# CarloLucibello/GraphNeuralNetworks.jl

Hardware: NVIDIA H100
Metric: edges/sec fwd+bwd GCNConv 128-dim on 100M-edge graph (higher is better)
Workload: dtype f32

## Files before the change

graphneuralnetworks.jl_b200/_lib.py:

```python
from __future__ import annotations

import ctypes as C
import os
import re

_HERE = os.path.dirname(os.path.abspath(__file__))
LIB_PATH = os.path.join(_HERE, "lib", "libgnnb200.so")
HEADER_PATH = os.path.join(os.path.dirname(_HERE), "include", "gnnb200.h")

OK, EINVAL, ESIZE, ECUDA, ENOMEM, EUNSUPPORTED, EINDEX = range(7)
COPY_XJ, W_MUL_XJ = 0, 1
SUM, MEAN, MAX, MIN = 0, 1, 2, 3
SRC, DST = 0, 1
DIR_OUT, DIR_IN, DIR_BOTH = 0, 1, 2
CODES_DIRECTED, CODES_DIRECTED_NOLOOP, CODES_UNDIRECTED, CODES_UNDIRECTED_NOLOOP, CODES_BIPARTITE = range(5)


class GNNBError(RuntimeError):

    def __init__(self, status: int, msg: str):
        super().__init__(f"libgnnb200 status {status}: {msg}")
        self.status = status


# ... 97 lines not shown
    "gnnb_edge_codes_sorted": (_int, [_int, _i64, _i64, _vp, _vp, _i64, _int, _vp, C.POINTER(_i64), _vp]),
    "gnnb_codes_member": (_int, [_vp, _i64, _vp, _i64, _vp, _vp]),
    "gnnb_sample_codes": (_int, [C.c_uint64, _vp, _i64, _i64, C.c_uint64, _vp, C.POINTER(_i64), _vp]),
    "gnnb_sample_positions_host": (_int, [_i32, _i64, _int, C.c_uint64, C.c_uint64, _vp, _i64, C.POINTER(_i64)]),
    "gnnb_propagate_host": (_int, [_vp, _int, _int, _int, _f32p, _f32p, _i64, _f32p]),
    "gnnb_gcn_propagate_host": (_int, [_vp, _int, _f32p, _f32p, _i64, _f32p]),
    "gnnb_linear2": (_int, [_f32p, _f32p, _f32p, _f32p, _int, _i64, _i64, _i64, _i64, _f32p, _vp]),
    "gnnb_linear2_bwd": (_int, [_f32p, _f32p, _f32p, _f32p, _f32p, _int, _i64, _i64, _i64, _i64, _f32p, _f32p, _f32p, _f32p, _f32p, _vp]),
    "gnnb_gat_logit_terms": (_int, [_f32p, _f32p, _i64, _i64, _i64, _f32p, _f32p, _vp]),
    "gnnb_gat_logit_terms_bwd": (_int, [_f32p, _f32p, _f32p, _f32p, _i64, _i64, _i64, _f32p, _f32p, _vp]),
    "gnnb_gcn_conv_step_host": (_int, [_vp, _vp, _vp, _vp, _int, _i64, _i64, _vp, _vp, _vp, _vp, _vp]),
    "gnnb_rmat_edges": (_int, [_i64, _i64, C.c_uint64, _vp, _vp, _vp]),
    "gnnb_rmat_edges_range": (_int, [_i64, _i64, _i64, C.c_uint64, _vp, _vp, _vp]),
    "gnnb_shard_builder_create": (_int, [C.POINTER(_vp), _i64, _int, _int, _int, C.POINTER(_i64), _vp]),
    "gnnb_shard_builder_add": (_int, [_vp, _vp, _vp, _i64, _int, _int, _vp]),
    "gnnb_shard_builder_finish": (_int, [_vp, _int, _int, C.POINTER(_vp), C.POINTER(_i64), C.POINTER(_i64), C.POINTER(_i64),
                                         C.POINTER(_i64), _vp]),
    "gnnb_degree_accumulate": (_int, [_vp, _vp, _i64, _int, _int, _i64, _vp, _vp]),
    "gnnb_balanced_relabel": (_int, [_vp, _i64, _int, _vp, _vp, _vp]),
    "gnnb_shard_builder_halo": (_int, [_vp, _int, _vp, _vp]),
    "gnnb_shard_builder_destroy": (_int, [_vp]),
    "gnnb_set_chunk_edges": (_int, [_int]),
    "gnnb_set_kernel_variant": (_int, [_int]),
}

for _name, (_res, _args) in _SIGS.items():
    _fn = getattr(lib, _name)
    _fn.restype = _res
    _fn.argtypes = _args


if os.environ.get("GNNB_KERNEL_VARIANT"):
    check(lib.gnnb_set_kernel_variant(int(os.environ["GNNB_KERNEL_VARIANT"])))


def device_count() -> int:
    return int(lib.gnnb_device_count())


def launch_count() -> int:
    return int(lib.gnnb_launch_count())


def version() -> str:
    return lib.gnnb_version().decode()
```

graphneuralnetworks.jl_b200/csrc/api.cu:

```cuda
#include "common.cuh"
#include <string.h>
#include <math_constants.h>

namespace gnnb {

static thread_local char t_err[512] = "";
std::atomic<int64_t> g_launches{0};

void set_error(const char* fmt, ...) {
    va_list ap;
    va_start(ap, fmt);
    vsnprintf(t_err, sizeof(t_err), fmt, ap);
    va_end(ap);
}

extern bool g_reference_kernels;
int edge_dot(gnnb_graph* g, const float* dout, const float* x, const float* cs, const float* ct, int64_t D,
             float* dw_coo, cudaStream_t st);
int maxmin_bwd(gnnb_graph* g, const float* w_plan_src, const float* x, const float* dout, const float* out_fwd,
               int64_t D, float* dx, cudaStream_t st);

__global__ void mul_vec_kernel(const float* __restrict__ a, const float* __restrict__ b, int64_t n, float* __restrict__ o) {
    int64_t i = (int64_t)blockIdx.x * blockDim.x + threadIdx.x;
    if (i < n) o[i] = a[i] * b[i];
}

__global__ void rmat_kernel(int64_t N, int64_t first, int64_t count, uint64_t seed, int scale, int64_t* __restrict__ src,
                            int64_t* __restrict__ dst) {
    const int64_t k = (int64_t)blockIdx.x * blockDim.x + threadIdx.x;
    if (k >= count) return;
    const int64_t id = first + k;
    const uint32_t TA = 9563013u, TB = 12750684u, TC = 15938355u;
    uint64_t s = 0, d = 0;
    for (uint64_t retry = 0;; ++retry) {
        uint64_t state = splitmix64(seed ^ splitmix64((uint64_t)id * 0x100000001B3ull + retry));
        s = 0; d = 0;
        for (int l = 0; l < scale; ++l) {
            state = splitmix64(state);
            const uint32_t u = (uint32_t)(state >> 40);
// ... 25 lines not shown

static int plan_weights(gnnb_graph* g, const Csr& c, int msg, const float* w, size_t ws2_off_floats, const float** out,
                        cudaStream_t st) {
    *out = nullptr;
    if (msg != GNNB_W_MUL_XJ || !w || g->E == 0) return GNNB_OK;
    GNNB_TRY(ensure_ws2(g, sizeof(float) * ((size_t)g->E + ws2_off_floats)));
    float* p = g->ws2 + ws2_off_floats;
    GNNB_TRY(permute_edge_values(c, g->E, w, 1, p, st));
    *out = p;
    return GNNB_OK;
}

extern "C" {

const char* gnnb_last_error(void) { return t_err; }
const char* gnnb_version(void) { return "gnnb200 0.1 sm_90a"; }
int gnnb_device_count(void) {
    int n = 0;
    if (cudaGetDeviceCount(&n) != cudaSuccess) { cudaGetLastError(); return 0; }
    return n;
}
int64_t gnnb_launch_count(void) { return g_launches.load(); }
int gnnb_set_kernel_variant(int v) {
    if (v != 0 && v != 12) GNNB_FAIL(GNNB_EINVAL, "kernel variant must be 0 (default) or 12 (reference kernels), got %d", v);
    gnnb::g_reference_kernels = v == 12;
    return GNNB_OK;
}

int gnnb_propagate(gnnb_graph_t g, int transposed, int msg, int aggr, const float* x, const float* w,
                   const float* cs, const float* ct, int64_t D, float* out, void* stream) {
    GNNB_TRY(check_common(g, msg, aggr, D, w));
    if (!x || !out) GNNB_FAIL(GNNB_EINVAL, "x/out is NULL");
    cudaStream_t st = (cudaStream_t)stream;
    GNNB_TRY(ensure_csr(g, transposed != 0, st));
    const Csr& c = transposed ? g->by_src : g->by_dst;
    SegArgs a;
    a.x = x; a.cs = cs; a.ct = ct; a.out = out; a.D = D; a.aggr = aggr;
    GNNB_TRY(plan_weights(g, c, msg, w, 0, &a.w, st));
    return seg_reduce(g, c, a, st);
}

int gnnb_propagate_bwd(gnnb_graph_t g, int msg, int aggr, const float* dout, const float* x, const float* w,
                       const float* cs, const float* ct, const float* out_fwd, int64_t D, float* dx, float* dw,
                       void* stream) {
    GNNB_TRY(check_common(g, msg, aggr, D, w));
    if (!dout) GNNB_FAIL(GNNB_EINVAL, "dout is NULL");
    cudaStream_t st = (cudaStream_t)stream;
    const bool ismax = aggr == GNNB_MAX || aggr == GNNB_MIN;
// ... 35 lines not shown
        if (!x) GNNB_FAIL(GNNB_EINVAL, "dw needs x");
        GNNB_TRY(edge_dot(g, dout, x, cs, gscale, D, dw, st));
    }
    return GNNB_OK;
}

int gnnb_gcn_propagate(gnnb_graph_t g, int transposed, const float* x, const float* w, const float* c,
                       int64_t D, float* out, void* stream) {
    if (!g) GNNB_FAIL(GNNB_EINVAL, "graph handle is NULL");
    if (g->n_src != g->n_dst) GNNB_FAIL(GNNB_ESIZE, "gcn_propagate needs num_src == num_dst");
    if (!c) {
        if (w) GNNB_FAIL(GNNB_EINVAL, "c is NULL: the plan-owned normalisation exists for unweighted graphs only");
        if (!x || !out) GNNB_FAIL(GNNB_EINVAL, "x/out is NULL");
        if (D <= 0) GNNB_FAIL(GNNB_ESIZE, "feature dimension must be positive (got %lld)", (long long)D);
        cudaStream_t st = (cudaStream_t)stream;
        GNNB_TRY(ensure_csr(g, transposed != 0, st));
        GNNB_TRY(ensure_gcn_scale(g, transposed != 0, st));
        const Csr& cc = transposed ? g->by_src : g->by_dst;
        SegArgs a;
        a.x = x; a.cs = g->gcn_c; a.es = cc.es; a.ct = g->gcn_c; a.out = out; a.D = D; a.aggr = GNNB_SUM;
        return seg_reduce(g, cc, a, st);
    }
    return gnnb_propagate(g, transposed, w ? GNNB_W_MUL_XJ : GNNB_COPY_XJ, GNNB_SUM, x, w, c, c, D, out, stream);
}

int gnnb_gcn_propagate_bipartite(gnnb_graph_t g, int transposed, const float* x, int64_t D, float* out, void* stream) {
    if (!g) GNNB_FAIL(GNNB_EINVAL, "graph handle is NULL");
    if (!x || !out) GNNB_FAIL(GNNB_EINVAL, "x/out is NULL");
    if (D <= 0) GNNB_FAIL(GNNB_ESIZE, "feature dimension must be positive (got %lld)", (long long)D);
    cudaStream_t st = (cudaStream_t)stream;
    GNNB_TRY(ensure_csr(g, transposed != 0, st));
    GNNB_TRY(ensure_bipartite_gcn_scale(g, transposed != 0, st));
    const Csr& cc = transposed ? g->by_src : g->by_dst;
    SegArgs a;
    a.x = x; a.out = out; a.D = D; a.aggr = GNNB_SUM;
    a.cs = transposed ? g->bip_c_dst : g->bip_c_src;
    a.es = transposed ? g->bip_es_src : g->bip_es_dst;
    a.ct = transposed ? g->bip_c_src : g->bip_c_dst;
    return seg_reduce(g, cc, a, st);
}

int gnnb_propagate_halo(gnnb_graph_t g, int msg, int aggr, const float* x_local, const float* x_halo,
                        int64_t n_local, const float* w, const float* cs, const float* ct, int64_t D, float* out,
                        void* stream) {
    GNNB_TRY(check_common(g, msg, aggr, D, w));
    if (!out) GNNB_FAIL(GNNB_EINVAL, "out is NULL");
// ... 165 lines not shown
```

graphneuralnetworks.jl_b200/csrc/common.cuh:

```cuda
#pragma once
#include <cuda_runtime.h>
#include <stdint.h>
#include <stdio.h>
#include <stdarg.h>
#include <atomic>
#include <mutex>
#include "../../include/gnnb200.h"

namespace gnnb {

void set_error(const char* fmt, ...);
extern std::atomic<int64_t> g_launches;

#define GNNB_CUDA(expr)                                                                   \
    do {                                                                                  \
        cudaError_t _e = (expr);                                                          \
        if (_e != cudaSuccess) {                                                          \
            ::gnnb::set_error("%s failed: %s (%s:%d)", #expr, cudaGetErrorString(_e),     \
                              __FILE__, __LINE__);                                        \
            return (_e == cudaErrorMemoryAllocation) ? GNNB_ENOMEM : GNNB_ECUDA;          \
        }                                                                                 \
    } while (0)

#define GNNB_TRY(expr)                 \
// ... 18 lines not shown

__host__ __device__ static inline uint64_t splitmix64(uint64_t x) {
    x += 0x9E3779B97F4A7C15ull;
    x = (x ^ (x >> 30)) * 0xBF58476D1CE4E5B9ull;
    x = (x ^ (x >> 27)) * 0x94D049BB133111EBull;
    return x ^ (x >> 31);
}

constexpr int kNumSMs = 132;

struct Csr {
    int32_t* rowptr = nullptr;
    int32_t* col = nullptr;
    int32_t* row = nullptr;
    int32_t* eid = nullptr;
    int32_t* long_rows = nullptr;
    int32_t n_long = 0;
    int32_t nrows = 0;
    float* invdeg = nullptr;
    int32_t* items = nullptr;
    int32_t n_items = 0;
    int32_t n_empty = -1;
    float* es = nullptr;
    bool built = false;
};

#ifdef __CUDACC__
__device__ __forceinline__ float fmax_nan(float a, float b) {
    float d;
    asm("max.NaN.f32 %0, %1, %2;" : "=f"(d) : "f"(a), "f"(b));
    return d;
}
__device__ __forceinline__ float softmax_shift(float Mn) { return Mn == -__int_as_float(0x7f800000) ? 0.f : Mn; }
#endif

}

struct gnnb_graph {
    int64_t E = 0;
    int32_t n_src = 0, n_dst = 0;
    int32_t chunk = 128;
    int device = 0;
    int32_t* coo_src = nullptr;
    int32_t* coo_dst = nullptr;
    gnnb::Csr by_dst;
    gnnb::Csr by_src;
    float* ws = nullptr;
    size_t ws_bytes = 0;
    float* ws2 = nullptr;
    size_t ws2_bytes = 0;
    float* gcn_c = nullptr;
    float* bip_c_src = nullptr;
    float* bip_c_dst = nullptr;
    float* bip_es_dst = nullptr;
    float* bip_es_src = nullptr;
    void* host_ws = nullptr;
    size_t host_ws_bytes = 0;
    std::mutex mu;
};

namespace gnnb {
int ensure_ws(gnnb_graph* g, size_t bytes);
int ensure_ws2(gnnb_graph* g, size_t bytes);
int ensure_csr(gnnb_graph* g, bool transposed, cudaStream_t st);
int ensure_invdeg(gnnb_graph* g, Csr& c, cudaStream_t st);
int ensure_items(gnnb_graph* g, const Csr& c, cudaStream_t st);
int ensure_gcn_scale(gnnb_graph* g, bool transposed, cudaStream_t st);
int ensure_bipartite_gcn_scale(gnnb_graph* g, bool transposed, cudaStream_t st);
int rsqrt_exact(float* d, int64_t n, cudaStream_t st);
int run_head_flags(const uint64_t* keys, int64_t E, int32_t* flags, cudaStream_t st);

struct SegArgs {
    const float* x = nullptr;
    const float* x2 = nullptr;
    int32_t split = 0;
    const float* w = nullptr;
    const float* cs = nullptr;
    const float* es = nullptr;
    const float* ct = nullptr;
    float* out = nullptr;
    int64_t D = 0;
    int aggr = GNNB_SUM;
};
int seg_reduce(gnnb_graph* g, const Csr& c, const SegArgs& a, cudaStream_t st);
int permute_edge_values(const Csr& c, int64_t E, const float* coo_vals, int64_t K, float* plan_vals,
                        cudaStream_t st);
int unpermute_edge_values(const Csr& c, int64_t E, const float* plan_vals, int64_t K,
                          float* coo_vals, cudaStream_t st);
}
```

graphneuralnetworks.jl_b200/csrc/plan.cu:

```cuda
#include "common.cuh"
#include <cub/cub.cuh>
#include <thrust/iterator/counting_iterator.h>
#include <thrust/iterator/transform_iterator.h>

namespace gnnb {

static int g_chunk_default = 128;

template <typename T>
__global__ void convert_index_kernel(const T* __restrict__ in, int64_t n, int64_t base, int64_t limit,
                                     int32_t* __restrict__ out, int* __restrict__ bad) {
    int64_t i = (int64_t)blockIdx.x * blockDim.x + threadIdx.x;
    if (i >= n) return;
    int64_t v = (int64_t)in[i] - base;
    if (v < 0 || v >= limit) {
        *bad = 1;
        v = 0;
    }
    out[i] = (int32_t)v;
}

__global__ void iota_kernel(int32_t* out, int64_t n, int32_t start) {
    int64_t i = (int64_t)blockIdx.x * blockDim.x + threadIdx.x;
    if (i < n) out[i] = start + (int32_t)i;
// ... 108 lines not shown
                                    const int32_t* __restrict__ eid, int64_t E, const int32_t* __restrict__ pos,
                                    const int32_t* __restrict__ newid, const int32_t* __restrict__ map,
                                    int32_t* __restrict__ nrow, int32_t* __restrict__ ncol,
                                    int32_t* __restrict__ neid) {
    int64_t k = (int64_t)blockIdx.x * blockDim.x + threadIdx.x;
    if (k >= E) return;
    const int32_t p = pos[k];
    if (pos[k + 1] == p) return;
    nrow[p] = map[row[k]];
    ncol[p] = map[col[k]];
    neid[p] = newid[eid[k]];
}

__global__ void bernoulli_keep_kernel(int64_t n, double p, uint64_t key, uint8_t* __restrict__ keep) {
    int64_t i = (int64_t)blockIdx.x * blockDim.x + threadIdx.x;
    if (i >= n) return;
    const double u = (double)(splitmix64(key + (uint64_t)i) >> 11) * 0x1.0p-53;
    keep[i] = (u < p) ? 0 : 1;
}

static void free_csr(Csr& c) {
    cudaFree(c.rowptr); cudaFree(c.col); cudaFree(c.row); cudaFree(c.eid);
    cudaFree(c.long_rows); cudaFree(c.invdeg); cudaFree(c.items); cudaFree(c.es);
    c = Csr();
}

static int alloc_csr(Csr& c, int64_t E, int32_t nrows, int32_t chunk) {
    c.nrows = nrows;
    GNNB_CUDA(cudaMalloc(&c.rowptr, sizeof(int32_t) * ((size_t)nrows + 1)));
    GNNB_CUDA(cudaMalloc(&c.col, sizeof(int32_t) * (size_t)(E > 0 ? E : 1)));
    GNNB_CUDA(cudaMalloc(&c.row, sizeof(int32_t) * (size_t)(E > 0 ? E : 1)));
    GNNB_CUDA(cudaMalloc(&c.eid, sizeof(int32_t) * (size_t)(E > 0 ? E : 1)));
    GNNB_CUDA(cudaMalloc(&c.long_rows, sizeof(int32_t) * (size_t)(E / chunk + 2)));
    return GNNB_OK;
}

static int find_long_rows(Csr& c, int32_t chunk, cudaStream_t st) {
    int32_t* d_count = nullptr;
    GNNB_CUDA(cudaMalloc(&d_count, sizeof(int32_t)));
    GNNB_CUDA(cudaMemsetAsync(d_count, 0, sizeof(int32_t), st));
    if (c.nrows > 0) {
        long_rows_kernel<<<(unsigned)ceil_div(c.nrows, 256), 256, 0, st>>>(c.rowptr, c.nrows, chunk,
                                                                           c.long_rows, d_count);
        GNNB_LAUNCHED();
    }
    GNNB_CUDA(cudaMemcpyAsync(&c.n_long, d_count, sizeof(int32_t), cudaMemcpyDeviceToHost, st));
// ... 376 lines not shown
```

graphneuralnetworks.jl_b200/csrc/seglean.cu:

```cuda
#include "common.cuh"
#include "segwalk.cuh"
#include <cub/cub.cuh>
#include <math_constants.h>

namespace gnnb {

struct LeanParams {
    const int4* __restrict__ items;
    const int32_t* __restrict__ col;
    const int32_t* __restrict__ row;
    const int32_t* __restrict__ rowptr;
    const float* __restrict__ es;
    const float* __restrict__ cs;
    const float* __restrict__ w;
    const float* __restrict__ ct;
    const float* __restrict__ x;
    const float* __restrict__ x2;
    float* __restrict__ out;
    float* __restrict__ ws;
    int32_t n_items;
    int32_t split;
    int32_t mean;
    float sign;
};

namespace {

__device__ __forceinline__ int chunk_items(const int32_t* __restrict__ rowptr, const int32_t* __restrict__ row, int64_t k,
                                           int C, int E, int nchunks, int4 out[3]) {
    const ChunkBounds b = chunk_bounds(rowptr, row, k, C, E, nchunks);
    if (b.e_begin >= b.e_end) return 0;
    int n = 0;
    int mb = b.e_begin, me = b.e_end;
    if (b.head_partial) {
        const int r0 = __ldg(row + b.e_begin);
        const int re0 = __ldg(rowptr + r0 + 1);
        const int hb = re0 < b.e_end ? re0 : b.e_end;
        out[n++] = make_int4(b.e_begin, hb, (int)(2 * k), 0);
        mb = hb;
    }
    int4 tail = make_int4(0, 0, -1, 0);
    if (mb < b.e_end && b.tail_partial) {
        const int r1 = __ldg(row + b.e_end - 1);
        const int rs1 = __ldg(rowptr + r1);
        const int tb = rs1 > mb ? rs1 : mb;
        me = tb;
// ... 33 lines not shown
    const int64_t r0 = ((int64_t)blockIdx.x * (blockDim.x >> 5) + (threadIdx.x >> 5)) * 32;
    const int64_t r = r0 + lane;
    const bool empty = r < nrows && __ldg(rowptr + r) == __ldg(rowptr + r + 1);
    unsigned m = __ballot_sync(0xffffffffu, empty);
    const float4 v4 = make_float4(v, v, v, v);
    while (m) {
        const int j = __ffs(m) - 1;
        m &= m - 1;
        float* base = out + (size_t)(r0 + j) * D;
        if ((D & 3) == 0 && (reinterpret_cast<uintptr_t>(base) & 15) == 0) {
            for (int64_t f = (int64_t)lane * 4; f < D; f += 128) *reinterpret_cast<float4*>(base + f) = v4;
        } else {
            for (int64_t f = lane; f < D; f += 32) base[f] = v;
        }
    }
}

__global__ void gather_scale_kernel(const int32_t* __restrict__ col, int64_t E, const float* __restrict__ c,
                                    float* __restrict__ es) {
    const int64_t e = (int64_t)blockIdx.x * blockDim.x + threadIdx.x;
    if (e < E) es[e] = __ldg(c + __ldg(col + e));
}

__device__ __forceinline__ float4 f4(float v) { return make_float4(v, v, v, v); }

constexpr int AG_SUM = 0, AG_MEAN = 1, AG_MAX = 2;

template <int SMODE, bool HAS_W, int AGG>
__device__ __forceinline__ float lcomb1(float acc, float v, float s1, float s2, float sign) {
    float m = v;
    if (SMODE != 0) m = __fmul_rn(m, s1);
    if (HAS_W) m = __fmul_rn(m, s2);
    if (AGG == AG_MAX) return fmax_nan(acc, __fmul_rn(m, sign));
    return __fadd_rn(acc, m);
}
template <int SMODE, bool HAS_W, int AGG>
__device__ __forceinline__ float4 lcomb(float4 a, float4 v, float s1, float s2, float sign) {
    return make_float4(lcomb1<SMODE, HAS_W, AGG>(a.x, v.x, s1, s2, sign), lcomb1<SMODE, HAS_W, AGG>(a.y, v.y, s1, s2, sign),
                       lcomb1<SMODE, HAS_W, AGG>(a.z, v.z, s1, s2, sign), lcomb1<SMODE, HAS_W, AGG>(a.w, v.w, s1, s2, sign));
}

template <int KV, int SMODE, bool HAS_W, int HALO, int AGG>
__global__ void __launch_bounds__(256, 4) seg_lean_kernel(const LeanParams p) {
    constexpr unsigned FULL = 0xffffffffu;
    constexpr int U = 8 / KV;
    constexpr int64_t STRIDE = (int64_t)KV * 128;
    const int lane = threadIdx.x & 31;
    const int item = blockIdx.x * 8 + (threadIdx.x >> 5);
    if (item >= p.n_items) return;
    const int4 it = __ldg(p.items + item);
    const int e_end = it.y;
    const bool partial = __any_sync(FULL, it.z >= 0);
    const float neutral = (AGG == AG_MAX) ? -CUDART_INF_F : 0.f;
    const float* const xl = p.x + lane * 4;
    const float* const x2l = HALO ? p.x2 + lane * 4 - (int64_t)p.split * STRIDE : nullptr;

    auto load_lane = [&](int e0, int& c, int& r, float& s1, float& s2, bool& last) {
        const int my = e0 + lane;
        c = 0; r = 0; s1 = 1.f; s2 = 1.f; last = false;
        if (my < e_end) {
            c = __ldg(p.col + my);
            r = __ldg(p.row + my);
            if (SMODE == 1) s1 = __ldg(p.es + my);
            if (HAS_W) s2 = __ldg(p.w + my);
            last = (my + 1 == e_end) || (__ldg(p.row + my + 1) != r);
            if (SMODE == 2) s1 = __ldg(p.cs + c);
        }
    };

    float4 acc[KV];
#pragma unroll
    for (int i = 0; i < KV; ++i) acc[i] = f4(neutral);

    int e = it.x;
    int c_n, r_n;
    float s1_n, s2_n;
    bool last_n;
    load_lane(e, c_n, r_n, s1_n, s2_n, last_n);
    bool more = true;
    while (more) {
        const int c_l = c_n, r_l = r_n;
        const float s1_l = s1_n, s2_l = s2_n;
        const unsigned vmask = __ballot_sync(FULL, e + lane < e_end);
        const unsigned bmask = partial ? 0u : __ballot_sync(FULL, last_n);
        float sc_l = 1.f, dg_l = 1.f;
        if (!partial && e + lane < e_end) {
            if (p.ct) sc_l = __ldg(p.ct + r_l);
            if (AGG == AG_MEAN) dg_l = (float)(__ldg(p.rowptr + r_l + 1) - __ldg(p.rowptr + r_l));
        }
        if (AGG == AG_MAX) sc_l *= p.sign;
        more = __any_sync(FULL, e + 32 < e_end);
        if (more) load_lane(e + 32, c_n, r_n, s1_n, s2_n, last_n);
#pragma unroll 1
        for (int j0 = 0; j0 < 32 && (vmask >> j0) != 0u; j0 += U) {
            float4 v[U][KV];
#pragma unroll
            for (int u = 0; u < U; ++u) {
                const int cj = __shfl_sync(FULL, c_l, j0 + u);
                const bool second = HALO != 0 && cj >= p.split;
                const float* xr = (second ? x2l : xl) + (int64_t)cj * STRIDE;
                if ((vmask >> (j0 + u)) & 1u) {
#pragma unroll
                    for (int i = 0; i < KV; ++i) v[u][i] = __ldg(reinterpret_cast<const float4*>(xr + i * 128));
                }
            }
#pragma unroll
            for (int u = 0; u < U; ++u) {
                const float s1 = (SMODE != 0) ? __shfl_sync(FULL, s1_l, j0 + u) : 1.f;
                const float s2 = HAS_W ? __shfl_sync(FULL, s2_l, j0 + u) : 1.f;
                if ((vmask >> (j0 + u)) & 1u) {
#pragma unroll
                    for (int i = 0; i < KV; ++i) acc[i] = lcomb<SMODE, HAS_W, AGG>(acc[i], v[u][i], s1, s2, p.sign);
                }
                if ((bmask >> (j0 + u)) & 1u) {
                    const int rj = __shfl_sync(FULL, r_l, j0 + u);
                    const float sc = __shfl_sync(FULL, sc_l, j0 + u);
                    float* o = p.out + (int64_t)rj * STRIDE + lane * 4;
                    if (AGG == AG_MEAN) {
                        const float dg = __shfl_sync(FULL, dg_l, j0 + u);
#pragma unroll
                        for (int i = 0; i < KV; ++i)
                            acc[i] = make_float4(__fdiv_rn(acc[i].x, dg), __fdiv_rn(acc[i].y, dg),
                                                 __fdiv_rn(acc[i].z, dg), __fdiv_rn(acc[i].w, dg));
                    }
#pragma unroll
                    for (int i = 0; i < KV; ++i) {
                        const float4 res = make_float4(acc[i].x * sc, acc[i].y * sc, acc[i].z * sc, acc[i].w * sc);
                        *reinterpret_cast<float4*>(o + i * 128) = res;
                        acc[i] = f4(neutral);
                    }
                }
            }
        }
        e += 32;
    }
    if (partial) {
        float* o = p.ws + (int64_t)it.z * STRIDE + lane * 4;
#pragma unroll
        for (int i = 0; i < KV; ++i) *reinterpret_cast<float4*>(o + i * 128) = acc[i];
    }
}

struct MaxBwdParams {
    const int4* __restrict__ items;
    const int32_t* __restrict__ col;
    const int32_t* __restrict__ row;
    const float* __restrict__ w;
    const float* __restrict__ x;
    const float* __restrict__ dout;
    const float* __restrict__ of;
    float* __restrict__ dx;
// ... 132 lines not shown
        LP(cub::DeviceScan::ExclusiveSum(nullptr, tmp_bytes, counts, offs, nchunks + 1, st));
        LP(cudaMalloc(&tmp, tmp_bytes ? tmp_bytes : 1));
        LP(cub::DeviceScan::ExclusiveSum(tmp, tmp_bytes, counts, offs, nchunks + 1, st));
        count_empty_rows_kernel<<<(unsigned)ceil_div((int64_t)c.nrows, 256), 256, 0, st>>>(c.rowptr, c.nrows, d_empty);
        int32_t n_items = 0, n_empty = 0;
        LP(cudaMemcpyAsync(&n_items, offs + nchunks, sizeof(int32_t), cudaMemcpyDeviceToHost, st));
        LP(cudaMemcpyAsync(&n_empty, d_empty, sizeof(int32_t), cudaMemcpyDeviceToHost, st));
        LP(cudaStreamSynchronize(st));
        LP(cudaMalloc(&items, sizeof(int4) * (size_t)(n_items > 0 ? n_items : 1)));
        item_emit_kernel<<<(unsigned)ceil_div(nchunks, 256), 256, 0, st>>>(c.rowptr, c.row, g->chunk, (int)g->E, nchunks, offs, items);
        LP(cudaGetLastError());
        LP(cudaStreamSynchronize(st));
        g_launches.fetch_add(4, std::memory_order_relaxed);
        mc.n_items = n_items;
        mc.n_empty = n_empty;
        mc.items = reinterpret_cast<int32_t*>(items);
        items = nullptr;
#undef LP
    } while (0);
    cudaFree(counts); cudaFree(offs); cudaFree(d_empty); cudaFree(tmp); cudaFree(items);
    return status;
}

int ensure_gcn_scale(gnnb_graph* g, bool transposed, cudaStream_t st) {
    Csr& c = transposed ? g->by_src : g->by_dst;
    if (g->gcn_c != nullptr && (c.es != nullptr || g->E == 0)) return GNNB_OK;
    if (g->gcn_c == nullptr) {
        float* buf = nullptr;
        GNNB_CUDA(cudaMalloc(&buf, sizeof(float) * (size_t)(g->n_dst > 0 ? g->n_dst : 1)));
        int rc = gnnb_gcn_norm(g, nullptr, buf, st);
        if (rc != GNNB_OK) { cudaFree(buf); return rc; }
        GNNB_CUDA(cudaStreamSynchronize(st));
        std::lock_guard<std::mutex> lock(g->mu);
        if (g->gcn_c == nullptr) g->gcn_c = buf; else cudaFree(buf);
    }
    if (c.es == nullptr && g->E > 0) {
        float* es = nullptr;
        GNNB_CUDA(cudaMalloc(&es, sizeof(float) * (size_t)g->E));
        gather_scale_kernel<<<(unsigned)ceil_div(g->E, 256), 256, 0, st>>>(c.col, g->E, g->gcn_c, es);
        GNNB_LAUNCHED();
        GNNB_CUDA(cudaStreamSynchronize(st));
        std::lock_guard<std::mutex> lock(g->mu);
        if (c.es == nullptr) c.es = es; else cudaFree(es);
    }
    return GNNB_OK;
}

int ensure_bipartite_gcn_scale(gnnb_graph* g, bool transposed, cudaStream_t st) {
    float*& es_slot = transposed ? g->bip_es_src : g->bip_es_dst;
    if (g->bip_c_src != nullptr && g->bip_c_dst != nullptr && (es_slot != nullptr || g->E == 0)) return GNNB_OK;
    GNNB_TRY(ensure_csr(g, true, st));
    if (g->bip_c_src == nullptr || g->bip_c_dst == nullptr) {
        float *cs = nullptr, *cd = nullptr;
        GNNB_CUDA(cudaMalloc(&cs, sizeof(float) * (size_t)(g->n_src > 0 ? g->n_src : 1)));
        GNNB_CUDA(cudaMalloc(&cd, sizeof(float) * (size_t)(g->n_dst > 0 ? g->n_dst : 1)));
        int rc = gnnb_degree(g, GNNB_DIR_OUT, nullptr, cs, st);
        if (rc == GNNB_OK) rc = gnnb_degree(g, GNNB_DIR_IN, nullptr, cd, st);
        if (rc == GNNB_OK) rc = rsqrt_exact(cs, g->n_src, st);
        if (rc == GNNB_OK) rc = rsqrt_exact(cd, g->n_dst, st);
        if (rc != GNNB_OK) { cudaFree(cs); cudaFree(cd); return rc; }
        GNNB_CUDA(cudaStreamSynchronize(st));
        std::lock_guard<std::mutex> lock(g->mu);
        if (g->bip_c_src == nullptr) { g->bip_c_src = cs; g->bip_c_dst = cd; } else { cudaFree(cs); cudaFree(cd); }
    }
    if (es_slot == nullptr && g->E > 0) {
        const Csr& c = transposed ? g->by_src : g->by_dst;
        float* es = nullptr;
// ... 11 lines not shown
    if (a.D != 128 && a.D != 256 && a.D != 512) return GNNB_EUNSUPPORTED;
    if ((reinterpret_cast<uintptr_t>(a.x) & 15) || (reinterpret_cast<uintptr_t>(a.x2) & 15) ||
        (reinterpret_cast<uintptr_t>(a.out) & 15))
        return GNNB_EUNSUPPORTED;
    const bool ismax = (a.aggr == GNNB_MAX || a.aggr == GNNB_MIN);
    const int agg = ismax ? AG_MAX : (a.aggr == GNNB_MEAN ? AG_MEAN : AG_SUM);
    const int smode = (a.cs == nullptr) ? 0 : (a.es != nullptr ? 1 : 2);
    const bool halo = a.x2 != nullptr;
    if (agg != AG_SUM && (smode != 0 || halo)) return GNNB_EUNSUPPORTED;
    GNNB_TRY(ensure_items(g, c, st));
    if (c.n_empty > 0) {
        const float v = a.aggr == GNNB_MAX ? -HUGE_VALF : (a.aggr == GNNB_MIN ? HUGE_VALF : 0.f);
        fill_empty_rows_warp_kernel<<<(unsigned)ceil_div((int64_t)c.nrows, 256), 256, 0, st>>>(c.rowptr, c.nrows, a.out, a.D, v);
        GNNB_LAUNCHED();
    }
    LeanParams p;
    p.items = reinterpret_cast<const int4*>(c.items);
    p.n_items = c.n_items;
    p.col = c.col; p.row = c.row; p.rowptr = c.rowptr;
    p.es = a.es; p.cs = a.cs; p.w = a.w; p.ct = a.ct;
    p.x = a.x; p.x2 = a.x2; p.split = a.split; p.out = a.out; p.ws = ws;
    p.mean = (a.aggr == GNNB_MEAN);
    p.sign = (a.aggr == GNNB_MIN) ? -1.f : 1.f;
    if (p.n_items == 0) return GNNB_OK;
    const int use_halo = halo ? 1 : 0;
    int rc;
    if (a.D == 128) rc = launch_lean1<1>(p, smode, a.w != nullptr, use_halo, agg, st);
    else if (a.D == 256) rc = launch_lean1<2>(p, smode, a.w != nullptr, use_halo, agg, st);
    else rc = launch_lean1<4>(p, smode, a.w != nullptr, use_halo, agg, st);
    return rc;
}

int seg_fixup_sum(const Csr& c, int64_t E, int chunk, int64_t D, float* ws, float* out, cudaStream_t st);
int maxmin_bwd_lean(gnnb_graph* g, const float* w_plan_src, const float* x, const float* dout, const float* out_fwd,
                    int64_t D, float* dx, cudaStream_t st) {
    if (D != 128 && D != 256 && D != 512) return GNNB_EUNSUPPORTED;
    if ((reinterpret_cast<uintptr_t>(x) & 15) || (reinterpret_cast<uintptr_t>(dout) & 15) ||
        (reinterpret_cast<uintptr_t>(out_fwd) & 15) || (reinterpret_cast<uintptr_t>(dx) & 15))
        return GNNB_EUNSUPPORTED;
    const Csr& c = g->by_src;
    if (g->E == 0) return GNNB_EUNSUPPORTED;
    GNNB_TRY(ensure_items(g, c, st));
    if (c.n_empty > 0) {
        fill_empty_rows_warp_kernel<<<(unsigned)ceil_div((int64_t)c.nrows, 256), 256, 0, st>>>(c.rowptr, c.nrows, dx, D, 0.f);
        GNNB_LAUNCHED();
    }
    MaxBwdParams p;
    p.items = reinterpret_cast<const int4*>(c.items);
    p.n_items = c.n_items;
    p.col = c.col; p.row = c.row; p.w = w_plan_src; p.x = x; p.dout = dout; p.of = out_fwd; p.dx = dx; p.ws = nullptr;
    if (c.n_long > 0) {
        GNNB_TRY(ensure_ws(g, (size_t)2 * ceil_div(g->E, g->chunk) * D * sizeof(float)));
// ... 16 lines not shown
```

include/gnnb200.h:

```cpp
#ifndef GNNB200_H
#define GNNB200_H

#include <stdint.h>

#ifdef __cplusplus
extern "C" {
#endif

typedef enum {
    GNNB_OK = 0,
    GNNB_EINVAL = 1,
    GNNB_ESIZE = 2,
    GNNB_ECUDA = 3,
    GNNB_ENOMEM = 4,
    GNNB_EUNSUPPORTED = 5,
    GNNB_EINDEX = 6
} gnnb_status;

typedef enum {
    GNNB_COPY_XJ = 0,
    GNNB_W_MUL_XJ = 1
} gnnb_msg;

typedef enum { GNNB_SUM = 0, GNNB_MEAN = 1, GNNB_MAX = 2, GNNB_MIN = 3 } gnnb_aggr;
// ... 30 lines not shown

int gnnb_degree(gnnb_graph_t g, int dir, const float* w, float* out, void* stream);

int gnnb_gather(gnnb_graph_t g, int which, const float* x, int64_t D, float* out, void* stream);

int gnnb_scatter(gnnb_graph_t g, int which, int aggr, const float* m, int64_t D, float* out,
                 void* stream);

int gnnb_propagate(gnnb_graph_t g, int transposed, int msg, int aggr, const float* x,
                   const float* w, const float* cs, const float* ct, int64_t D, float* out,
                   void* stream);

int gnnb_propagate_bwd(gnnb_graph_t g, int msg, int aggr, const float* dout, const float* x,
                       const float* w, const float* cs, const float* ct, const float* out_fwd,
                       int64_t D, float* dx, float* dw, void* stream);

int gnnb_softmax_edge_neighbors(gnnb_graph_t g, const float* e, int64_t K, float* out, void* stream);
int gnnb_softmax_edge_neighbors_bwd(gnnb_graph_t g, const float* alpha, const float* dalpha,
                                    int64_t K, float* de, void* stream);

int gnnb_gcn_norm(gnnb_graph_t g, const float* w, float* c_out, void* stream);
int gnnb_gcn_propagate(gnnb_graph_t g, int transposed, const float* x, const float* w,
                       const float* c, int64_t D, float* out, void* stream);
int gnnb_gcn_propagate_bipartite(gnnb_graph_t g, int transposed, const float* x, int64_t D, float* out, void* stream);

int gnnb_gat_aggregate(gnnb_graph_t g, const float* Wx, const float* el, const float* er,
                       int64_t C, int64_t H, float slope, float* out, float* alpha,
                       float* seg_max, float* seg_sum, void* stream);
int gnnb_gat_aggregate_bwd(gnnb_graph_t g, const float* Wx, const float* el, const float* er,
                           const float* seg_max, const float* seg_sum, const float* out_fwd,
                           const float* dout, int64_t C, int64_t H, float slope, float* dWx, float* del,
                           float* der, void* stream);

int gnnb_gat_logit_terms(const float* Wx, const float* a, int64_t N, int64_t C, int64_t H, float* el, float* er, void* stream);
int gnnb_gat_logit_terms_bwd(const float* Wx, const float* a, const float* del, const float* der, int64_t N, int64_t C,
                             int64_t H, float* dWx_accum, float* da, void* stream);

int gnnb_linear(const float* x, const float* W, const float* bias, int relu, int64_t N, int64_t Din,
                int64_t Dout, float* y, void* stream);
int gnnb_linear_bwd(const float* dy, const float* y, const float* x, const float* W, int relu, int64_t N,
                    int64_t Din, int64_t Dout, float* dpre_ws, float* dx, float* dW, float* db, void* stream);
int gnnb_linear_relu_mask(const float* x, const float* W, const float* bias, int64_t N, int64_t Din, int64_t Dout, float* y,
                          uint32_t* mask, void* stream);
int gnnb_linear_bwd_mask(const float* dy, const uint32_t* mask, const float* x, const float* W, int64_t N, int64_t Din,
                         int64_t Dout, float* dx, float* dW, float* db, void* stream);
int gnnb_linear2(const float* x1, const float* x2, const float* W, const float* bias, int relu, int64_t N, int64_t Din1,
// ... 133 lines not shown
```

Measured before the change: 2.096 billion.

## Pin high-degree source rows in L2 with cache-policy hints during GCN gather

During GCN scale setup, the code counts how often each source row is gathered, picks a threshold so the hottest rows fit in about half of L2, and marks those edges by setting the sign bit of the per-edge scale. In the 128-dim lean seg-reduce kernel, gathers of hot rows use an evict_last policy, cold rows use evict_first, and output stores use evict_first. A follow-up kernel resets the hot rows to evict_normal. The aim is to cut DRAM traffic from repeated gathers on power-law graphs, in exchange for a one-time count/sort/sync setup, an extra launch per propagate, and a sign-bit encoding trick on the edge scales.

```diff
diff --git a/graphneuralnetworks.jl_b200/_lib.py b/graphneuralnetworks.jl_b200/_lib.py
--- a/graphneuralnetworks.jl_b200/_lib.py
+++ b/graphneuralnetworks.jl_b200/_lib.py
@@ -143,6 +143,7 @@
     "gnnb_shard_builder_destroy": (_int, [_vp]),
     "gnnb_set_chunk_edges": (_int, [_int]),
     "gnnb_set_kernel_variant": (_int, [_int]),
+    "gnnb_gcn_hot_rows": (_int, [_vp, _int, _vp, _i64, C.POINTER(_i64), C.POINTER(C.c_int32), _vp]),
 }
 
 for _name, (_res, _args) in _SIGS.items():
diff --git a/graphneuralnetworks.jl_b200/csrc/api.cu b/graphneuralnetworks.jl_b200/csrc/api.cu
--- a/graphneuralnetworks.jl_b200/csrc/api.cu
+++ b/graphneuralnetworks.jl_b200/csrc/api.cu
@@ -15,6 +15,7 @@
 }
 
 extern bool g_reference_kernels;
+extern bool g_l2_policy_forced;
 int edge_dot(gnnb_graph* g, const float* dout, const float* x, const float* cs, const float* ct, int64_t D,
              float* dw_coo, cudaStream_t st);
 int maxmin_bwd(gnnb_graph* g, const float* w_plan_src, const float* x, const float* dout, const float* out_fwd,
@@ -86,8 +87,10 @@
 }
 int64_t gnnb_launch_count(void) { return g_launches.load(); }
 int gnnb_set_kernel_variant(int v) {
-    if (v != 0 && v != 12) GNNB_FAIL(GNNB_EINVAL, "kernel variant must be 0 (default) or 12 (reference kernels), got %d", v);
+    if (v != 0 && v != 12 && v != 14)
+        GNNB_FAIL(GNNB_EINVAL, "kernel variant must be 0 (default), 12 (reference kernels) or 14 (L2 policy at every size), got %d", v);
     gnnb::g_reference_kernels = v == 12;
+    gnnb::g_l2_policy_forced = v == 14;
     return GNNB_OK;
 }
 
@@ -169,6 +172,14 @@
         return seg_reduce(g, cc, a, st);
     }
     return gnnb_propagate(g, transposed, w ? GNNB_W_MUL_XJ : GNNB_COPY_XJ, GNNB_SUM, x, w, c, c, D, out, stream);
+}
+
+int gnnb_gcn_hot_rows(gnnb_graph_t g, int transposed, int32_t* rows_host, int64_t capacity, int64_t* num_rows,
+                      int32_t* threshold, void* stream) {
+    if (!g) GNNB_FAIL(GNNB_EINVAL, "graph handle is NULL");
+    if (g->n_src != g->n_dst) GNNB_FAIL(GNNB_ESIZE, "gcn_hot_rows needs num_src == num_dst");
+    if (capacity < 0) GNNB_FAIL(GNNB_ESIZE, "capacity must be >= 0");
+    return gcn_hot_rows(g, transposed != 0, rows_host, capacity, num_rows, threshold, (cudaStream_t)stream);
 }
 
 int gnnb_gcn_propagate_bipartite(gnnb_graph_t g, int transposed, const float* x, int64_t D, float* out, void* stream) {
diff --git a/graphneuralnetworks.jl_b200/csrc/common.cuh b/graphneuralnetworks.jl_b200/csrc/common.cuh
--- a/graphneuralnetworks.jl_b200/csrc/common.cuh
+++ b/graphneuralnetworks.jl_b200/csrc/common.cuh
@@ -64,6 +64,9 @@
     int32_t n_items = 0;
     int32_t n_empty = -1;
     float* es = nullptr;
+    int32_t hot_min = 0;
+    int32_t* hot_rows = nullptr;
+    int32_t n_hot = 0;
     bool built = false;
 };
 
@@ -108,6 +111,8 @@
 int ensure_invdeg(gnnb_graph* g, Csr& c, cudaStream_t st);
 int ensure_items(gnnb_graph* g, const Csr& c, cudaStream_t st);
 int ensure_gcn_scale(gnnb_graph* g, bool transposed, cudaStream_t st);
+int gcn_hot_rows(gnnb_graph* g, bool transposed, int32_t* rows_host, int64_t capacity, int64_t* num_rows,
+                 int32_t* threshold, cudaStream_t st);
 int ensure_bipartite_gcn_scale(gnnb_graph* g, bool transposed, cudaStream_t st);
 int rsqrt_exact(float* d, int64_t n, cudaStream_t st);
 int run_head_flags(const uint64_t* keys, int64_t E, int32_t* flags, cudaStream_t st);
diff --git a/graphneuralnetworks.jl_b200/csrc/plan.cu b/graphneuralnetworks.jl_b200/csrc/plan.cu
--- a/graphneuralnetworks.jl_b200/csrc/plan.cu
+++ b/graphneuralnetworks.jl_b200/csrc/plan.cu
@@ -154,6 +154,7 @@
 static void free_csr(Csr& c) {
     cudaFree(c.rowptr); cudaFree(c.col); cudaFree(c.row); cudaFree(c.eid);
     cudaFree(c.long_rows); cudaFree(c.invdeg); cudaFree(c.items); cudaFree(c.es);
+    cudaFree(c.hot_rows);
     c = Csr();
 }
 
diff --git a/graphneuralnetworks.jl_b200/csrc/seglean.cu b/graphneuralnetworks.jl_b200/csrc/seglean.cu
--- a/graphneuralnetworks.jl_b200/csrc/seglean.cu
+++ b/graphneuralnetworks.jl_b200/csrc/seglean.cu
@@ -22,6 +22,7 @@
     int32_t split;
     int32_t mean;
     float sign;
+    int32_t l2hint;
 };
 
 namespace {
@@ -101,9 +102,58 @@
     if (e < E) es[e] = __ldg(c + __ldg(col + e));
 }
 
+__global__ void count_gathers_kernel(const int32_t* __restrict__ col, int64_t E, int32_t* __restrict__ cnt) {
+    const int64_t e = (int64_t)blockIdx.x * blockDim.x + threadIdx.x;
+    if (e < E) atomicAdd(cnt + __ldg(col + e), 1);
+}
+__global__ void flag_hot_kernel(const int32_t* __restrict__ col, int64_t E, const int32_t* __restrict__ cnt, int32_t t,
+                                float* __restrict__ es) {
+    const int64_t e = (int64_t)blockIdx.x * blockDim.x + threadIdx.x;
+    if (e < E && __ldg(cnt + __ldg(col + e)) >= t) es[e] = __uint_as_float(__float_as_uint(es[e]) | 0x80000000u);
+}
+__global__ void list_hot_kernel(const int32_t* __restrict__ cnt, int32_t n, int32_t t, int32_t* __restrict__ rows,
+                                int32_t* __restrict__ n_rows) {
+    const int64_t j = (int64_t)blockIdx.x * blockDim.x + threadIdx.x;
+    if (j < n && cnt[j] >= t) rows[atomicAdd(n_rows, 1)] = (int32_t)j;
+}
+__global__ void demote_rows_kernel(const int32_t* __restrict__ rows, int32_t n_rows, const float* __restrict__ x) {
+    const int64_t i = (int64_t)blockIdx.x * blockDim.x + threadIdx.x;
+    if (i >= (int64_t)n_rows * 4) return;
+    const float* line = x + (int64_t)__ldg(rows + (i >> 2)) * 128 + (i & 3) * 32;
+    asm volatile("applypriority.global.L2::evict_normal [%0], 128;" :: "l"(line) : "memory");
+}
+
 __device__ __forceinline__ float4 f4(float v) { return make_float4(v, v, v, v); }
 
 constexpr int AG_SUM = 0, AG_MEAN = 1, AG_MAX = 2;
+
+constexpr int L2_HOT_LAST = 1, L2_COLD_FIRST = 2, L2_OUT_FIRST = 4;
+
+__device__ __forceinline__ uint64_t policy_evict_last() {
+    uint64_t pol;
+    asm("createpolicy.fractional.L2::evict_last.b64 %0, 1.0;" : "=l"(pol));
+    return pol;
+}
+__device__ __forceinline__ uint64_t policy_evict_first() {
+    uint64_t pol;
+    asm("createpolicy.fractional.L2::evict_first.b64 %0, 1.0;" : "=l"(pol));
+    return pol;
+}
+__device__ __forceinline__ uint64_t policy_evict_normal() {
+    uint64_t pol;
+    asm("createpolicy.fractional.L2::evict_normal.b64 %0, 1.0;" : "=l"(pol));
+    return pol;
+}
+__device__ __forceinline__ float4 ldg_policy(const float* ptr, uint64_t pol) {
+    float4 v;
+    asm("ld.global.nc.L2::cache_hint.v4.f32 {%0, %1, %2, %3}, [%4], %5;"
+        : "=f"(v.x), "=f"(v.y), "=f"(v.z), "=f"(v.w) : "l"(ptr), "l"(pol));
+    return v;
+}
+__device__ __forceinline__ void st_policy(float* ptr, float4 v, uint64_t pol) {
+    asm volatile("st.global.L2::cache_hint.v4.f32 [%0], {%1, %2, %3, %4}, %5;"
+                 :: "l"(ptr), "f"(v.x), "f"(v.y), "f"(v.z), "f"(v.w), "l"(pol) : "memory");
+}
 
 template <int SMODE, bool HAS_W, int AGG>
 __device__ __forceinline__ float lcomb1(float acc, float v, float s1, float s2, float sign) {
@@ -150,6 +200,12 @@
     float4 acc[KV];
 #pragma unroll
     for (int i = 0; i < KV; ++i) acc[i] = f4(neutral);
+    constexpr bool HINTS = SMODE == 1 && KV == 1 && HALO == 0;
+    uint64_t pol_hot = 0, pol_cold = 0;
+    if (HINTS && p.l2hint) {
+        pol_hot = (p.l2hint & L2_HOT_LAST) ? policy_evict_last() : policy_evict_normal();
+        pol_cold = (p.l2hint & L2_COLD_FIRST) ? policy_evict_first() : policy_evict_normal();
+    }
 
     int e = it.x;
     int c_n, r_n;
@@ -162,6 +218,7 @@
         const float s1_l = s1_n, s2_l = s2_n;
         const unsigned vmask = __ballot_sync(FULL, e + lane < e_end);
         const unsigned bmask = partial ? 0u : __ballot_sync(FULL, last_n);
+        const unsigned hmask = HINTS ? __ballot_sync(FULL, __float_as_int(s1_l) < 0) : 0u;
         float sc_l = 1.f, dg_l = 1.f;
         if (!partial && e + lane < e_end) {
             if (p.ct) sc_l = __ldg(p.ct + r_l);
@@ -179,13 +236,20 @@
                 const bool second = HALO != 0 && cj >= p.split;
                 const float* xr = (second ? x2l : xl) + (int64_t)cj * STRIDE;
                 if ((vmask >> (j0 + u)) & 1u) {
-#pragma unroll
-                    for (int i = 0; i < KV; ++i) v[u][i] = __ldg(reinterpret_cast<const float4*>(xr + i * 128));
+                    if (HINTS && p.l2hint) {
+                        const uint64_t pol = ((hmask >> (j0 + u)) & 1u) ? pol_hot : pol_cold;
+#pragma unroll
+                        for (int i = 0; i < KV; ++i) v[u][i] = ldg_policy(xr + i * 128, pol);
+                    } else {
+#pragma unroll
+                        for (int i = 0; i < KV; ++i) v[u][i] = __ldg(reinterpret_cast<const float4*>(xr + i * 128));
+                    }
                 }
             }
 #pragma unroll
             for (int u = 0; u < U; ++u) {
-                const float s1 = (SMODE != 0) ? __shfl_sync(FULL, s1_l, j0 + u) : 1.f;
+                const float s1 = SMODE == 1 ? __int_as_float(__shfl_sync(FULL, __float_as_int(s1_l), j0 + u) & 0x7fffffff)
+                                            : (SMODE != 0) ? __shfl_sync(FULL, s1_l, j0 + u) : 1.f;
                 const float s2 = HAS_W ? __shfl_sync(FULL, s2_l, j0 + u) : 1.f;
                 if ((vmask >> (j0 + u)) & 1u) {
 #pragma unroll
@@ -205,7 +269,8 @@
 #pragma unroll
                     for (int i = 0; i < KV; ++i) {
                         const float4 res = make_float4(acc[i].x * sc, acc[i].y * sc, acc[i].z * sc, acc[i].w * sc);
-                        *reinterpret_cast<float4*>(o + i * 128) = res;
+                        if (HINTS && (p.l2hint & L2_OUT_FIRST)) st_policy(o + i * 128, res, policy_evict_first());
+                        else *reinterpret_cast<float4*>(o + i * 128) = res;
                         acc[i] = f4(neutral);
                     }
                 }
@@ -384,6 +449,66 @@
     return status;
 }
 
+bool g_l2_policy_forced = false;
+
+constexpr double kHotL2Fraction = 0.56;
+constexpr int64_t kL2PolicyMinRatio = 8;
+constexpr int kL2Hints = L2_HOT_LAST | L2_COLD_FIRST | L2_OUT_FIRST;
+
+static int l2_bytes(const gnnb_graph* g, int64_t* bytes) {
+    int v = 0;
+    GNNB_CUDA(cudaDeviceGetAttribute(&v, cudaDevAttrL2CacheSize, g->device));
+    *bytes = v;
+    return GNNB_OK;
+}
+
+static int flag_hot_rows(gnnb_graph* g, Csr& c, int32_t n, float* es, int32_t* t_out, int32_t** rows_out,
+                         int32_t* n_rows_out, cudaStream_t st) {
+    int64_t l2 = 0;
+    GNNB_TRY(l2_bytes(g, &l2));
+    int64_t budget = (int64_t)((double)l2 * kHotL2Fraction) / 512;
+    int32_t *cnt = nullptr, *sorted = nullptr, *rows = nullptr, *d_nrows = nullptr;
+    void* tmp = nullptr;
+    int status = GNNB_OK;
+    do {
+#define LP(expr) { cudaError_t _e = (expr); if (_e != cudaSuccess) { set_error("%s failed: %s", #expr, cudaGetErrorString(_e)); status = (_e == cudaErrorMemoryAllocation) ? GNNB_ENOMEM : GNNB_ECUDA; break; } }
+        LP(cudaMalloc(&cnt, sizeof(int32_t) * (size_t)n));
+        LP(cudaMemsetAsync(cnt, 0, sizeof(int32_t) * (size_t)n, st));
+        count_gathers_kernel<<<(unsigned)ceil_div(g->E, 256), 256, 0, st>>>(c.col, g->E, cnt);
+        LP(cudaGetLastError());
+        int32_t t = 1;
+        if (n > budget) {
+            size_t tmp_bytes = 0;
+            LP(cudaMalloc(&sorted, sizeof(int32_t) * (size_t)n));
+            LP(cub::DeviceRadixSort::SortKeysDescending(nullptr, tmp_bytes, cnt, sorted, n, 0, 32, st));
+            LP(cudaMalloc(&tmp, tmp_bytes ? tmp_bytes : 1));
+            LP(cub::DeviceRadixSort::SortKeysDescending(tmp, tmp_bytes, cnt, sorted, n, 0, 32, st));
+            int32_t kth = 0;
+            LP(cudaMemcpyAsync(&kth, sorted + budget, sizeof(int32_t), cudaMemcpyDeviceToHost, st));
+            LP(cudaStreamSynchronize(st));
+            t = kth + 1;
+        }
+        flag_hot_kernel<<<(unsigned)ceil_div(g->E, 256), 256, 0, st>>>(c.col, g->E, cnt, t, es);
+        LP(cudaGetLastError());
+        LP(cudaMalloc(&rows, sizeof(int32_t) * (size_t)(n < budget ? n : budget)));
+        LP(cudaMalloc(&d_nrows, sizeof(int32_t)));
+        LP(cudaMemsetAsync(d_nrows, 0, sizeof(int32_t), st));
+        list_hot_kernel<<<(unsigned)ceil_div(n, 256), 256, 0, st>>>(cnt, n, t, rows, d_nrows);
+        LP(cudaGetLastError());
+        int32_t n_rows = 0;
+        LP(cudaMemcpyAsync(&n_rows, d_nrows, sizeof(int32_t), cudaMemcpyDeviceToHost, st));
+        LP(cudaStreamSynchronize(st));
+        g_launches.fetch_add(n > budget ? 4 : 3, std::memory_order_relaxed);
+        *t_out = t;
+        *rows_out = rows;
+        *n_rows_out = n_rows;
+        rows = nullptr;
+#undef LP
+    } while (0);
+    cudaFree(cnt); cudaFree(sorted); cudaFree(tmp); cudaFree(rows); cudaFree(d_nrows);
+    return status;
+}
+
 int ensure_gcn_scale(gnnb_graph* g, bool transposed, cudaStream_t st) {
     Csr& c = transposed ? g->by_src : g->by_dst;
     if (g->gcn_c != nullptr && (c.es != nullptr || g->E == 0)) return GNNB_OK;
@@ -401,10 +526,25 @@
         GNNB_CUDA(cudaMalloc(&es, sizeof(float) * (size_t)g->E));
         gather_scale_kernel<<<(unsigned)ceil_div(g->E, 256), 256, 0, st>>>(c.col, g->E, g->gcn_c, es);
         GNNB_LAUNCHED();
-        GNNB_CUDA(cudaStreamSynchronize(st));
+        int32_t t = 0, n_hot = 0;
+        int32_t* hot = nullptr;
+        const int rc = flag_hot_rows(g, c, transposed ? g->n_dst : g->n_src, es, &t, &hot, &n_hot, st);
+        if (rc != GNNB_OK) { cudaFree(es); return rc; }
         std::lock_guard<std::mutex> lock(g->mu);
-        if (c.es == nullptr) c.es = es; else cudaFree(es);
-    }
+        if (c.es == nullptr) { c.es = es; c.hot_min = t; c.hot_rows = hot; c.n_hot = n_hot; } else { cudaFree(es); cudaFree(hot); }
+    }
+    return GNNB_OK;
+}
+
+int gcn_hot_rows(gnnb_graph* g, bool transposed, int32_t* rows_host, int64_t capacity, int64_t* num_rows,
+                 int32_t* threshold, cudaStream_t st) {
+    GNNB_TRY(ensure_csr(g, transposed, st));
+    GNNB_TRY(ensure_gcn_scale(g, transposed, st));
+    const Csr& c = transposed ? g->by_src : g->by_dst;
+    if (num_rows) *num_rows = c.n_hot;
+    if (threshold) *threshold = c.hot_min;
+    const int64_t n = capacity < c.n_hot ? capacity : c.n_hot;
+    if (rows_host && n > 0) GNNB_CUDA(cudaMemcpy(rows_host, c.hot_rows, sizeof(int32_t) * (size_t)n, cudaMemcpyDeviceToHost));
     return GNNB_OK;
 }
 
@@ -462,12 +602,22 @@
     p.x = a.x; p.x2 = a.x2; p.split = a.split; p.out = a.out; p.ws = ws;
     p.mean = (a.aggr == GNNB_MEAN);
     p.sign = (a.aggr == GNNB_MIN) ? -1.f : 1.f;
+    p.l2hint = 0;
+    if (smode == 1 && a.es == c.es && c.hot_min > 0 && a.D == 128 && !halo) {
+        int64_t l2 = 0;
+        GNNB_TRY(l2_bytes(g, &l2));
+        if (g_l2_policy_forced || (int64_t)g->n_src * a.D * 4 >= kL2PolicyMinRatio * l2) p.l2hint = kL2Hints;
+    }
     if (p.n_items == 0) return GNNB_OK;
     const int use_halo = halo ? 1 : 0;
     int rc;
     if (a.D == 128) rc = launch_lean1<1>(p, smode, a.w != nullptr, use_halo, agg, st);
     else if (a.D == 256) rc = launch_lean1<2>(p, smode, a.w != nullptr, use_halo, agg, st);
     else rc = launch_lean1<4>(p, smode, a.w != nullptr, use_halo, agg, st);
+    if (rc == GNNB_OK && (p.l2hint & L2_HOT_LAST) && c.n_hot > 0) {
+        demote_rows_kernel<<<(unsigned)ceil_div((int64_t)c.n_hot * 4, 256), 256, 0, st>>>(c.hot_rows, c.n_hot, a.x);
+        GNNB_LAUNCHED();
+    }
     return rc;
 }
 
diff --git a/include/gnnb200.h b/include/gnnb200.h
--- a/include/gnnb200.h
+++ b/include/gnnb200.h
@@ -76,6 +76,8 @@
 int gnnb_gcn_norm(gnnb_graph_t g, const float* w, float* c_out, void* stream);
 int gnnb_gcn_propagate(gnnb_graph_t g, int transposed, const float* x, const float* w,
                        const float* c, int64_t D, float* out, void* stream);
+int gnnb_gcn_hot_rows(gnnb_graph_t g, int transposed, int32_t* rows_host, int64_t capacity, int64_t* num_rows,
+                      int32_t* threshold, void* stream);
 int gnnb_gcn_propagate_bipartite(gnnb_graph_t g, int transposed, const float* x, int64_t D, float* out, void* stream);
 
 int gnnb_gat_aggregate(gnnb_graph_t g, const float* Wx, const float* el, const float* er,
```

Result: faster. 2.245 billion (median of 6 runs) (+7.1%).
